# enricobottazzi/zk-fhe

Hardware: AMD Instinct MI355X
Metric: BFV proofs/sec (k=13) (higher is better)
Workload: dtype u32x8 (256-bit Montgomery integers over BN254 Fr/Fq)

## Files before the change

### zk-fhe_amd/csrc/msm.hip

```cpp
#include <cstdio>
#include <vector>
#include <cstring>

#include "ctx.hpp"
#include "fq29.hip.hpp"
#include "g1x29_wave.hip.hpp"

using namespace zk;

namespace {


__device__ __forceinline__ bool fr_gt_half(const Fr &s) {
  const u32 H[8] = {0xf8000000u, 0xa1f0fac9u, 0x3cdcb848u, 0x9419f424u, 0x40c0ac2eu, 0xdc2822dbu, 0x7098d014u, 0x18322739u};
#pragma unroll
  for (int i = 7; i >= 0; --i) {
    if (s.l[i] > H[i]) return true;
    if (s.l[i] < H[i]) return false;
  }
  return false;
}

struct Digits {
  int c, windows;
};

template <class F>
__device__ __forceinline__ void for_each_digit(const Fr &mont, int c, int windows, F f) {
  Fr s = fp_from_mont<FrP>(mont);
  bool neg = fr_gt_half(s);
  if (neg) s = fp_neg<FrP>(s);
  u32 carry = 0;
  const u32 mask = (1u << c) - 1, halfv = 1u << (c - 1);
  for (int w = 0; w < windows; ++w) {
    u32 v = (s.l[0] & mask) + carry;
#pragma unroll
    for (int i = 0; i < 7; ++i) s.l[i] = __builtin_amdgcn_alignbit(s.l[i + 1], s.l[i], (u32)c);
    s.l[7] >>= c;
    bool dneg = false;
    if (v > halfv) {
      v = (1u << c) - v;
      dneg = true;
      carry = 1;
    } else {
      carry = 0;
    }
    if (v) f(w, v, neg != dneg);
  }
}

constexpr size_t MSM_MAX_COLS = 4096;
constexpr unsigned SORT_CHUNK = 2048;
constexpr unsigned SORT_THREADS = 512;

__global__ void __launch_bounds__(SORT_THREADS) k_msm_hist(const Fr *__restrict__ scalars, size_t col_stride, size_t n, unsigned chunks_per_col, int c, int windows,
                                                          unsigned *__restrict__ hist , unsigned K1) {
  extern __shared__ unsigned lh[];
  const size_t col = blockIdx.x / chunks_per_col;
  const unsigned chunk = blockIdx.x % chunks_per_col;
  for (unsigned b = threadIdx.x; b < K1; b += SORT_THREADS) lh[b] = 0;
  __syncthreads();
  const size_t i0 = (size_t)chunk * SORT_CHUNK, i1 = min(n, i0 + SORT_CHUNK);
  for (size_t i = i0 + threadIdx.x; i < i1; i += SORT_THREADS)
    for_each_digit(scalars[col * col_stride + i], c, windows, [&](int, u32 b, bool) { atomicAdd(&lh[b], 1u); });
  __syncthreads();
  unsigned *h = hist + col * K1;
  for (unsigned b = threadIdx.x; b < K1; b += SORT_THREADS) {
    const unsigned v = lh[b];
    if (v) atomicAdd(&h[b], v);
  }
}

__global__ void __launch_bounds__(256) k_msm_scan(const unsigned *__restrict__ hist, unsigned *__restrict__ off,
                                                  unsigned *__restrict__ cursor, unsigned K1) {
  __shared__ unsigned part[256];
  const unsigned *h = hist + (size_t)blockIdx.x * K1;
  unsigned *o = off + (size_t)blockIdx.x * K1;
  unsigned *cu = cursor + (size_t)blockIdx.x * K1;
  const unsigned K = K1 - 1;
  const unsigned per = (K + 255) / 256;
  const unsigned lo = threadIdx.x * per, hi = min(lo + per, K);
  unsigned s = 0;
  for (unsigned b = lo; b < hi; ++b) s += h[b + 1];
  part[threadIdx.x] = s;
  __syncthreads();
  if (threadIdx.x == 0) {
    unsigned acc = 0;
    for (int i = 0; i < 256; ++i) {
      unsigned t = part[i];
      part[i] = acc;
      acc += t;
    }
  }
  __syncthreads();
  unsigned acc = part[threadIdx.x];
  for (unsigned b = lo; b < hi; ++b) {
    o[b] = acc;
    cu[b + 1] = acc;
    acc += h[b + 1];
  }
  if (hi == K) o[K] = acc;
}

__global__ void __launch_bounds__(SORT_THREADS) k_msm_scatter(const Fr *__restrict__ scalars, size_t col_stride, size_t n, unsigned chunks_per_col, int c, int windows,
                                                             unsigned *__restrict__ cursor, unsigned K1, unsigned *__restrict__ entries,
                                                             size_t col_entries) {
  extern __shared__ unsigned lh[];
  const size_t col = blockIdx.x / chunks_per_col;
  const unsigned chunk = blockIdx.x % chunks_per_col;
  for (unsigned b = threadIdx.x; b < K1; b += SORT_THREADS) lh[b] = 0;
  __syncthreads();
  const size_t i0 = (size_t)chunk * SORT_CHUNK, i1 = min(n, i0 + SORT_CHUNK);
  for (size_t i = i0 + threadIdx.x; i < i1; i += SORT_THREADS)
    for_each_digit(scalars[col * col_stride + i], c, windows, [&](int, u32 b, bool) { atomicAdd(&lh[b], 1u); });
  __syncthreads();
  unsigned *cu = cursor + col * K1;
  for (unsigned b = threadIdx.x; b < K1; b += SORT_THREADS) {
    const unsigned v = lh[b];
    lh[b] = v ? atomicAdd(&cu[b], v) : 0u;
  }
  __syncthreads();
  unsigned *e = entries + col * col_entries;
  for (size_t i = i0 + threadIdx.x; i < i1; i += SORT_THREADS)
    for_each_digit(scalars[col * col_stride + i], c, windows, [&](int w, u32 b, bool neg) {
      const unsigned pos = atomicAdd(&lh[b], 1u);
      e[pos] = ((unsigned)w * (unsigned)n + (unsigned)i) | (neg ? 0x80000000u : 0u);
    });
}

constexpr unsigned CH_SCALARS = 2048, CS_SCALARS = 512, CS_THREADS = 256, FINE_THREADS = 512, FINE_MAX = 256, FINE_COPIES = 8, FINE_CTRS = FINE_MAX * FINE_COPIES, FINE_TILE = 14336;
static_assert(FINE_CTRS == 4 * FINE_THREADS && FINE_TILE % (4 * FINE_THREADS) == 0, "k_msm_fine: four counters per thread, whole 16-byte loads per tile");
constexpr int FINE_BITS_MAX = 8;

__global__ void __launch_bounds__(CS_THREADS) k_msm_chist(const Fr *__restrict__ scalars, size_t col_stride, size_t n, unsigned chunks_per_col, int c, int windows,
                                                         int L, unsigned NB, unsigned *__restrict__ chist ) {
  extern __shared__ unsigned lh[];
  const size_t col = blockIdx.x / chunks_per_col;
  const unsigned chunk = blockIdx.x % chunks_per_col;
  for (unsigned b = threadIdx.x; b < NB; b += CS_THREADS) lh[b] = 0;
  __syncthreads();
  const size_t i0 = (size_t)chunk * CH_SCALARS, i1 = min(n, i0 + CH_SCALARS);
  for (size_t i = i0 + threadIdx.x; i < i1; i += CS_THREADS)
    for_each_digit(scalars[col * col_stride + i], c, windows, [&](int, u32 b, bool) { atomicAdd(&lh[(b - 1) >> L], 1u); });
  __syncthreads();
  for (unsigned g = threadIdx.x; g < NB; g += CS_THREADS) {
    const unsigned v = lh[g];
    if (v) atomicAdd(&chist[col * NB + g], v);
  }
}

__global__ void __launch_bounds__(64) k_msm_cscan(const unsigned *__restrict__ chist, unsigned NB, size_t n_cols, unsigned *__restrict__ coff ,
                                                  unsigned *__restrict__ ccursor ) {
  const size_t col = blockIdx.x * (size_t)blockDim.x + threadIdx.x;
  if (col >= n_cols) return;
  unsigned acc = 0;
  for (unsigned g = 0; g < NB; ++g) {
    coff[col * (NB + 1) + g] = acc;
    ccursor[col * NB + g] = acc;
    acc += chist[col * NB + g];
// ... 337 lines not shown
      const unsigned h = base + (lane >> 3), sub = lane & 7;
      size_t g = 0;
      unsigned nt = 0, pa = 0, pb = 0;
      Slices s = {0, 0, 0};
      if (h < cnt) {
        g = medium_list[h];
        const size_t col = g / K;
        const unsigned b = (unsigned)(g - col * K);
        const unsigned *o = off + col * (K + 1);
        s = slices_of(o[b + 1] - o[b], TASK_E);
        nt = s.nt;
        pa = bucket_posA[g];
        pb = bucket_posB[g];
      }
      G1X29 acc = G1X29::identity();
      for (unsigned j = sub; j < nt; j += 8) g1x29_add(acc, g1x29_load(partials[partial_pos(s, pa, pb, j)]));
      for (int m = 1; m < 8; m <<= 1) {
        const G1X29 other = g1x_shfl_xor(acc, m);
        g1x29_add(acc, other);
      }
      if (nt && sub == 0) buckets[g] = g1x29_store(acc);
    }
    return;
  }
  const unsigned first = large_blocks + medium_blocks, light_blocks = gridDim.x - first;
  const size_t total = (size_t)K * n_cols;
  for (size_t g = (blockIdx.x - first) * (size_t)blockDim.x + threadIdx.x; g < total; g += (size_t)light_blocks * blockDim.x) {
    const size_t col = g / K;
    const unsigned b = (unsigned)(g - col * K);
    const unsigned *o = off + col * (K + 1);
    const Slices s = slices_of(o[b + 1] - o[b], TASK_E);
    const unsigned nt = s.nt;
    if (nt > (unsigned)MERGE_LIGHT) continue;
    G1X first = G1X::identity();
    if (nt) {
      const unsigned pa = bucket_posA[g], pb = bucket_posB[g];
      first = partials[partial_pos(s, pa, pb, 0)];
      if (nt > 1) {
        G1X29 acc = g1x29_load(first);
        G1X nxt = partials[partial_pos(s, pa, pb, 1)];
        for (unsigned j = 1; j < nt; ++j) {
          const G1X cur = nxt;
          if (j + 1 < nt) nxt = partials[partial_pos(s, pa, pb, j + 1)];
          g1x29_add(acc, g1x29_load(cur));
        }
        first = g1x29_store(acc);
      }
    }
    buckets[g] = first;
  }
}

__device__ __forceinline__ G1X g1x_mul_pow2(G1X p, int k) {
  for (int i = 0; i < k; ++i) p = g1x_dbl(p);
  return p;
}
__device__ __forceinline__ G1X29 g1x29_mul_pow2(G1X29 p, int k) {
  for (int i = 0; i < k; ++i) p = g1x29_dbl(p);
  return p;
}

__global__ void __launch_bounds__(256) k_msm_marginals(const G1X *__restrict__ buckets, unsigned K, size_t n_cols, unsigned L ,
                                                       unsigned w0, unsigned w_cnt ,
                                                       G1X *__restrict__ marg ) {
  const unsigned A = K >> 6;
  const unsigned per_col = A + 64;
  const unsigned G = 64 / L;
  const size_t wave = (blockIdx.x * (size_t)blockDim.x + threadIdx.x) >> 6;
  const unsigned lane = threadIdx.x & 63, g = lane & (G - 1), sub = lane / G;
  const size_t o = wave * G + g;
  const bool live = o < n_cols * w_cnt;
  const size_t col = live ? o / w_cnt : 0;
  const unsigned w = w0 + (unsigned)(o - col * w_cnt);
  const G1X *B = buckets + col * K;
  size_t base, stride;
  unsigned cnt;
  if (w < A) {
    base = (size_t)w * 64 + sub;
    stride = L;
    cnt = 64 / L;
  } else {
    base = (size_t)sub * 64 + (w - A);
    stride = (size_t)L * 64;
    cnt = A > sub ? (A - sub + L - 1) / L : 0;
  }
  if (!live) cnt = 0;
  G1X29 v = G1X29::identity();
  for (unsigned i = 0; i < cnt; ++i) g1x29_add(v, g1x29_load(B[base + i * stride]));
  for (int m = (int)G; m < 64; m <<= 1) {
    const G1X29 other = g1x_shfl_xor(v, m);
    g1x29_add(v, other);
  }
  if (live && sub == 0) marg[col * per_col + w] = g1x29_store(v);
}

template <bool XYZZ>
__global__ void __launch_bounds__(576) k_msm_weighted(const G1X *__restrict__ marg, unsigned K, void *__restrict__ out) {
  __shared__ G1X sh[9];
  const unsigned A = K >> 6;
  const unsigned row_waves = (A + 63) / 64;
  const size_t col = blockIdx.x;
  const unsigned lane = threadIdx.x & 63, wv = threadIdx.x >> 6;
  const G1X *M = marg + col * (A + 64);
  const bool rows = wv < row_waves;
  const unsigned a = wv * 64 + lane;
  const G1X29 P = g1x29_load(rows ? (a < A ? M[a] : G1X::identity()) : M[A + lane]);
  const unsigned k = rows ? a : lane + 1;
  int nbits = 7;
  if (rows) {
    nbits = 0;
    while ((1u << nbits) < A) ++nbits;
  }
  G1X29 W = G1X29::identity();
  for (int bit = nbits - 1; bit >= 0; --bit) {
    W = g1x29_dbl(W);
    if ((k >> bit) & 1) g1x29_add(W, P);
  }
  if (rows) W = g1x29_mul_pow2(W, 6);
  for (int m = 1; m < 64; m <<= 1) {
    const G1X29 other = g1x_shfl_xor(W, m);
    g1x29_add(W, other);
  }
  if (lane == 0) sh[wv] = g1x29_store(W);
  __syncthreads();
  if (threadIdx.x == 0) {
    G1X29 t = g1x29_load(sh[0]);
    for (unsigned w = 1; w <= row_waves; ++w) g1x29_add(t, g1x29_load(sh[w]));
    if (XYZZ) ((G1X *)out)[col] = g1x29_to_std(t);
    else ((G1Affine *)out)[col] = g1x_to_affine(g1x29_to_std(t));
  }
}

template <bool XYZZ>
__global__ void __launch_bounds__(64) k_msm_small(const G1X *__restrict__ buckets, unsigned K, void *__restrict__ out) {
  const size_t col = blockIdx.x;
  const unsigned lane = threadIdx.x;
  const G1X29 P = g1x29_load(lane < K ? buckets[col * K + lane] : G1X::identity());
  const unsigned k = lane + 1;
  G1X29 W = G1X29::identity();
  for (int bit = 6; bit >= 0; --bit) {
    W = g1x29_dbl(W);
    if ((k >> bit) & 1) g1x29_add(W, P);
  }
  for (int m = 1; m < 64; m <<= 1) {
    const G1X29 other = g1x_shfl_xor(W, m);
    g1x29_add(W, other);
  }
  if (lane == 0) {
    if (XYZZ) ((G1X *)out)[col] = g1x29_to_std(W);
    else ((G1Affine *)out)[col] = g1x_to_affine(g1x29_to_std(W));
  }
}

struct BiasArg {
  u32 l[9];
};

__device__ __forceinline__ u32 bits_at(const u32 (&l)[9], int bit, int c) {
  const int limb = bit >> 5, sh = bit & 31;
  u32 lo = 0, hi = 0;
#pragma unroll
  for (int k = 0; k < 9; ++k) {
    if (k == limb) lo = l[k];
    if (k == limb + 1) hi = l[k];
  }
  return (u32)((((u64)hi << 32) | lo) >> sh) & ((1u << c) - 1);
}

__device__ __forceinline__ bool biased_scalar(const Fr &mont, const BiasArg &B, u32 (&out)[9], int &bits) {
  Fr s = fp_from_mont<FrP>(mont);
  const bool neg = fr_gt_half(s);
  if (neg) s = fp_neg<FrP>(s);
  bits = 0;
#pragma unroll
  for (int k = 0; k < 8; ++k)
    if (s.l[k]) bits = 32 * k + 32 - __clz(s.l[k]);
  u32 carry = 0;
#pragma unroll
  for (int k = 0; k < 8; ++k) {
    const u64 v = (u64)s.l[k] + B.l[k] + carry;
    out[k] = (u32)v;
    carry = (u32)(v >> 32);
  }
  out[8] = B.l[8] + carry;
  return neg;
}

__global__ void __launch_bounds__(64) k_basis_multiples(const G1Affine *__restrict__ bases, size_t n, int c, int W, G1Affine *__restrict__ T) {
  const size_t t = blockIdx.x * (size_t)blockDim.x + threadIdx.x;
  if (t >= n * (size_t)W) return;
  const size_t i = t / (size_t)W;
  const int w = (int)(t % (size_t)W);
  const size_t J = (size_t)1 << (c - 1);
  G1Affine *row = T + t * J;
  G1Affine b = bases[i];
  if (!b.is_identity() && w) b = g1x_to_affine(g1x_mul_pow2(g1x_from_affine(b), c * w));
  if (b.is_identity()) {
    for (size_t j = 0; j < J; ++j) row[j] = b;
    return;
  }
  row[0] = g1_affine_to_29(b);
  if (J == 1) return;
  G1X acc = g1x_from_affine_dbl(b);
  row[1] = g1_affine_to_29(g1x_to_affine(acc));
  for (size_t j = 2; j < J; ++j) {
    g1x_add_affine(acc, b, false);
    row[j] = g1_affine_to_29(g1x_to_affine(acc));
  }
}

template <bool TREE>
__global__ void __launch_bounds__(256, TREE ? 1 : 3) k_msm_table(const Fr *__restrict__ scalars, size_t col_stride, size_t n, const G1Affine *__restrict__ T, int c, int W, BiasArg B,
                                                   unsigned P, unsigned cpc , unsigned n_cols, unsigned max_part,
                                                   G1X *__restrict__ partials ,
                                                   unsigned *__restrict__ n_part ,
                                                   unsigned *__restrict__ col_next ,
                                                   unsigned *__restrict__ lists , unsigned long long *__restrict__ adds) {
  unsigned *__restrict__ lst = lists + (size_t)blockIdx.x * P * (unsigned)W;
  __shared__ G1X sh[TREE ? 128 : 1];
  __shared__ unsigned wave_cnt[4], item_sh;
  const unsigned lane = threadIdx.x & 63, wv = threadIdx.x >> 6;
  const int half = 1 << (c - 1);
  G1X29 acc = G1X29::identity();
  unsigned col = (unsigned)(((unsigned long long)blockIdx.x * n_cols) / gridDim.x), done = 0, total = 0;
  for (;;) {
    __syncthreads();
    if (threadIdx.x == 0) item_sh = atomicAdd(&col_next[col], 1u);
    __syncthreads();
    const unsigned chunk = item_sh;
    if (chunk >= cpc) {
      if (done) {
        if (TREE) acc = block_sum_256(acc, sh);
        __syncthreads();
        if (threadIdx.x == 0) item_sh = atomicAdd(&n_part[col], 1u);
        __syncthreads();
        const size_t slot = (size_t)col * max_part + item_sh;
        if (TREE) {
          if (threadIdx.x == 0) partials[slot] = g1x29_store(acc);
        } else {
          partials[slot * 256 + threadIdx.x] = g1x29_store(acc);
        }
        acc = G1X29::identity();
        done = 0;
      }
      __syncthreads();
      if (threadIdx.x == 0) item_sh = 0;
      __syncthreads();
      const unsigned MIN_JOIN = cpc < 4u ? cpc : 4u;
      unsigned best = 0;
      for (unsigned j = threadIdx.x; j < n_cols; j += 256) {
        const unsigned nx = __hip_atomic_load(&col_next[j], __ATOMIC_RELAXED, __HIP_MEMORY_SCOPE_AGENT);
        if (nx < cpc && (nx == 0 || cpc - nx >= MIN_JOIN)) {
          const unsigned h = ((j * 2654435761u) ^ (blockIdx.x * 40503u + 12345u) * 2246822519u) >> 13;
          best = max(best, (((h & 0x7ffffu) + 1u) << 12) | j);
        }
      }
      if (best) atomicMax(&item_sh, best);
      __syncthreads();
      const unsigned found = item_sh;
      if (!found) break;
      col = found & 4095u;
      continue;
    }
    ++done;
    {
      const size_t i = (size_t)chunk * P + threadIdx.x;
      const bool valid = threadIdx.x < P && i < n;
      u32 sb[9];
      bool neg = false;
      unsigned long long mask = 0;
      if (valid) {
        int bits;
        neg = biased_scalar(scalars[(size_t)col * col_stride + i], B, sb, bits);
        const int wtop = min(W, bits / c + 2);
        for (int w = 0; w < wtop; ++w)
          if ((int)bits_at(sb, w * c, c) != half) mask |= 1ull << w;
      }
      const unsigned mine = (unsigned)__popcll(mask);
      unsigned incl = mine;
#pragma unroll
      for (int d = 1; d < 64; d <<= 1) {
        const unsigned t = __shfl_up(incl, d);
        if ((int)lane >= d) incl += t;
      }
      if (lane == 63) wave_cnt[wv] = incl;
      __syncthreads();
      unsigned off = incl - mine;
      for (unsigned v = 0; v < wv; ++v) off += wave_cnt[v];
      const unsigned row0 = threadIdx.x * (unsigned)W;
      while (mask) {
        const int w = __builtin_ctzll(mask);
        mask &= mask - 1;
        const int d = (int)bits_at(sb, w * c, c) - half;
        lst[off++] = (((row0 + (unsigned)w) << (c - 1)) + (unsigned)(d < 0 ? -d : d) - 1u) | ((neg != (d < 0)) ? 0x80000000u : 0u);
      }
    }
    __syncthreads();
    const unsigned M = wave_cnt[0] + wave_cnt[1] + wave_cnt[2] + wave_cnt[3];
    total += M;
    const G1Affine *__restrict__ Tc = T + (((size_t)chunk * P * (size_t)W) << (c - 1));
    unsigned e = threadIdx.x, en = 0, en2 = 0;
    G1Affine p;
    if (e < M) {
      en = lst[e];
      p = Tc[en & 0x7fffffffu];
    }
    if (e + 256 < M) en2 = lst[e + 256];
    while (e < M) {
      const unsigned e2 = e + 256;
      unsigned en3 = 0;
      G1Affine p2;
      if (e2 < M) p2 = Tc[en2 & 0x7fffffffu];
      if (e2 + 256 < M) en3 = lst[e2 + 256];
      g1x29_add_affine(acc, g1a29_load(p), (en >> 31) != 0);
      e = e2;
      en = en2;
      en2 = en3;
      p = p2;
    }
  }
  if (adds && threadIdx.x == 0 && total) atomicAdd(adds, (unsigned long long)total);
}

template <bool XYZZ>
__global__ void __launch_bounds__(512) k_msm_table_fold(const G1X *__restrict__ partials, unsigned max_part, unsigned L, unsigned *__restrict__ n_part,
                                                        unsigned *__restrict__ col_next, void *__restrict__ out) {
  __shared__ G1X sh[256];
  const unsigned col = blockIdx.x, t = threadIdx.x & 255u, q = threadIdx.x >> 8;
  const unsigned np = n_part[col] * L;
  const G1X *mine = partials + (size_t)col * max_part * L;
  G1X29 f = G1X29::identity();
  {
    const unsigned first = L == 256 ? q * 256u + t : threadIdx.x, step = 512u;
    unsigned b = first;
    G1X cur;
    if (b < np) cur = mine[b];
    while (b < np) {
      const unsigned nb = b + step;
      G1X nxt;
      if (nb < np) nxt = mine[nb];
      g1x29_add(f, g1x29_load(cur));
      cur = nxt;
      b = nb;
    }
  }
  if (q == 1) sh[t] = g1x29_store(f);
  __syncthreads();
  if (q == 0) g1x29_add(f, g1x29_load(sh[t]));
  __syncthreads();
  if (q == 0 && t >= 128) sh[t - 128] = g1x29_store(f);
  __syncthreads();
  if (q == 0 && t < 128) g1x29_add(f, g1x29_load(sh[t]));
  __syncthreads();
  if (q == 0 && t >= 64 && t < 128) sh[t - 64] = g1x29_store(f);
  __syncthreads();
  if (threadIdx.x < 64) {
    g1x29_add(f, g1x29_load(sh[t]));
    for (int m = 1; m < 64; m <<= 1) {
      const G1X29 other = g1x_shfl_xor(f, m);
      g1x29_add(f, other);
    }
    if (threadIdx.x == 0) {
      if (XYZZ) ((G1X *)out)[col] = g1x29_to_std(f);
      else ((G1Affine *)out)[col] = g1x_to_affine(g1x29_to_std(f));
      n_part[col] = 0;
      col_next[col] = 0;
    }
  }
}

__global__ void __launch_bounds__(256) k_basis_table(const G1Affine *__restrict__ bases, size_t n, int c, int windows,
                                                     G1Affine *__restrict__ table) {
  const size_t i = blockIdx.x * (size_t)blockDim.x + threadIdx.x;
  if (i >= n) return;
  G1Affine p = bases[i];
  table[i] = g1_affine_to_29(p);
  G1X cur = g1x_from_affine(p);
  for (int w = 1; w < windows; ++w) {
    cur = g1x_mul_pow2(cur, c);
    G1Affine a = g1x_to_affine(cur);
    table[(size_t)w * n + i] = g1_affine_to_29(a);
    cur = g1x_from_affine(a);
  }
}

__global__ void __launch_bounds__(256) k_g1_add(const G1Affine *__restrict__ a, const G1Affine *__restrict__ b,
                                                G1Affine *__restrict__ out, size_t n) {
  const size_t i = blockIdx.x * (size_t)blockDim.x + threadIdx.x;
  if (i >= n) return;
  G1X acc = g1x_from_affine(a[i]);
  g1x_add_affine(acc, b[i], false);
  out[i] = g1x_to_affine(acc);
}

__global__ void __launch_bounds__(256) k_g1_mul(const G1Affine *__restrict__ p, const Fr *__restrict__ k,
                                                G1Affine *__restrict__ out, size_t n) {
  const size_t i = blockIdx.x * (size_t)blockDim.x + threadIdx.x;
  if (i >= n) return;
  const Fr s = fp_from_mont<FrP>(k[i]);
  const G1Affine base = p[i];
  G1X acc = G1X::identity();
  for (int bit = 255; bit >= 0; --bit) {
    acc = g1x_dbl(acc);
    if ((s.l[bit >> 5] >> (bit & 31)) & 1) g1x_add_affine(acc, base, false);
  }
  out[i] = g1x_to_affine(acc);
}

template <bool XYZZ>
__global__ void __launch_bounds__(64) k_msm_sparse(const zkfhe_sparse_term *__restrict__ terms, unsigned n_terms, const G1Affine *__restrict__ T, int c, int W,
                                                   BiasArg B, void *__restrict__ out) {
  const unsigned slot = blockIdx.x, lane = threadIdx.x;
  const int half = 1 << (c - 1);
  G1X29 acc = G1X29::identity();
  for (unsigned t = 0; t < n_terms; ++t) {
    if (terms[t].slot != slot) continue;
    Fr s;
#pragma unroll
    for (int i = 0; i < 4; ++i) {
      s.l[2 * i] = (u32)terms[t].scalar.l[i];
      s.l[2 * i + 1] = (u32)(terms[t].scalar.l[i] >> 32);
    }
    u32 sb[9];
    int bits;
    const bool neg = biased_scalar(s, B, sb, bits);
    const int d = (int)lane < W ? (int)bits_at(sb, (int)lane * c, c) - half : 0;
    if (d) {
      const G1Affine p = T[(((size_t)terms[t].row * W + lane) << (c - 1)) + (size_t)(d < 0 ? -d : d) - 1];
      g1x29_add_affine(acc, g1a29_load(p), neg != (d < 0));
    }
  }
  for (int m = 1; m < 64; m <<= 1) {
    const G1X29 other = g1x_shfl_xor(acc, m);
    g1x29_add(acc, other);
  }
  if (lane == 0) {
    if (XYZZ) ((G1X *)out)[slot] = g1x29_to_std(acc);
    else ((G1Affine *)out)[slot] = g1x_to_affine(g1x29_to_std(acc));
  }
}

int table_bits(size_t n, double budget_scale) {
  const char *e = getenv("ZKFHE_TABLE_BITS");
  const int forced = e ? atoi(e) : -1;
  const char *g = getenv("ZKFHE_TABLE_GB");
  double gb = g ? atof(g) : 48.0;
  if (!g) {
    size_t free_b = 0, total_b = 0;
    if (hipMemGetInfo(&free_b, &total_b) == hipSuccess && (double)free_b / 4.0 < gb * 1073741824.0) gb = (double)free_b / 4.0 / 1073741824.0;
  }
  const double budget = gb * 1073741824.0 * budget_scale;
  auto fits = [&](int c) {
    const double entries = (double)n * (double)((255 + c - 1) / c) * (double)(1u << (c - 1));
    return c >= 8 && c <= 15 && entries * sizeof(G1Affine) <= budget;
  };
  if (forced >= 0) return forced > 0 && fits(forced) ? forced : 0;
  for (int c = 15; c >= 8; --c)
    if (fits(c)) return c;
  return 0;
}

size_t table_reserve_bytes(size_t total_b) {
  if (const char *r = getenv("ZKFHE_TABLE_RESERVE_GB")) return (size_t)(atof(r) * 1073741824.0);
  const size_t eighth = total_b / 8, floor_b = (size_t)24 << 30;
  return eighth > floor_b ? eighth : floor_b;
}

BiasArg table_bias(int c, int W) {
  BiasArg B;
  memset(&B, 0, sizeof(B));
  for (int w = 0; w < W; ++w) {
    const int bit = c * w + c - 1;
    B.l[bit >> 5] |= 1u << (bit & 31);
  }
  return B;
}

int msm_table(zkfhe_ctx *ctx, const zkfhe_basis *basis, const Fr *scalars, size_t col_stride, size_t n_cols, void *out, bool xyzz) {
  const size_t n = basis->n;
  const int c = basis->mc, W = basis->mw;
  const size_t words = 2 * MSM_MAX_COLS + 4;
  if (!ctx->tickets) {
    ZK_HIP(ctx, hipMalloc((void **)&ctx->tickets, words * sizeof(unsigned)));
    ZK_HIP(ctx, zk_memset_async(ctx, ctx->tickets, 0, words * sizeof(unsigned), ctx->stream));
  }
  unsigned *n_part = ctx->tickets, *col_next = ctx->tickets + MSM_MAX_COLS;
  unsigned long long *adds = (unsigned long long *)(ctx->tickets + 2 * MSM_MAX_COLS);
  const size_t grid_max = (size_t)ctx->num_cu * 3;
  size_t P = 256;
  while (P > 128 && n_cols * ((n + P - 1) / P) < grid_max) P >>= 1;
  const size_t cpc = (n + P - 1) / P, n_items = n_cols * cpc;
  const size_t grid = n_items < grid_max ? n_items : grid_max;
  const size_t max_part = cpc < grid ? cpc : grid;
  const bool tree = n_cols <= 16;
  const unsigned L = tree ? 1 : 256;
  void *p0, *p1;
  int rc = zk_scratch(ctx, 0, n_cols * max_part * L * sizeof(G1X), &p0);
  if (rc) return rc;
  rc = zk_scratch(ctx, 1, grid * P * (size_t)W * 4, &p1);
  if (rc) return rc;
  const bool big = n_cols * n > ((size_t)1 << 16);
  const int slot = big ? 0 : 2;
  if (ctx->prof_on) ZK_HIP(ctx, zk_memset_async(ctx, adds, 0, 8, ctx->stream));
  zk_prof_begin(ctx);
  if (tree)
    k_msm_table<true><<<(unsigned)grid, 256, 0, ctx->stream>>>(scalars, col_stride, n, basis->mult, c, W, table_bias(c, W), (unsigned)P, (unsigned)cpc, (unsigned)n_cols,
                                                             (unsigned)max_part, (G1X *)p0, n_part, col_next, (unsigned *)p1, ctx->prof_on ? adds : nullptr);
  else
    k_msm_table<false><<<(unsigned)grid, 256, 0, ctx->stream>>>(scalars, col_stride, n, basis->mult, c, W, table_bias(c, W), (unsigned)P, (unsigned)cpc, (unsigned)n_cols,
                                                              (unsigned)max_part, (G1X *)p0, n_part, col_next, (unsigned *)p1, ctx->prof_on ? adds : nullptr);
  ZK_LAUNCH_CHECK(ctx);
  zk_prof_end(ctx, slot, 96.0 * (double)n * (double)n_cols);
  {
    static const bool dbg = getenv("ZKFHE_DEBUG_NPART") != nullptr;
    if (dbg) {
      std::vector<unsigned> np(n_cols);
      ZK_HIP(ctx, hipMemcpy(np.data(), n_part, n_cols * sizeof(unsigned), hipMemcpyDeviceToHost));
      unsigned long long sum = 0;
      unsigned mx = 0;
      for (unsigned v : np) {
        sum += v;
        mx = v > mx ? v : mx;
      }
      fprintf(stderr, "[msm_table] cols %zu  chunks/col %zu  grid %zu  visits/col avg %.1f max %u\n", n_cols, cpc, grid, (double)sum / n_cols, mx);
    }
  }
  if (xyzz) k_msm_table_fold<true><<<(unsigned)n_cols, 512, 0, ctx->stream>>>((const G1X *)p0, (unsigned)max_part, L, n_part, col_next, out);
  else k_msm_table_fold<false><<<(unsigned)n_cols, 512, 0, ctx->stream>>>((const G1X *)p0, (unsigned)max_part, L, n_part, col_next, out);
  ZK_LAUNCH_CHECK(ctx);
  if (ctx->prof_on) {
    unsigned long long h = 0;
    ZK_HIP(ctx, hipMemcpy(&h, adds, 8, hipMemcpyDeviceToHost));
    ctx->prof_ops[slot] += (double)h;
  }
  return ZKFHE_OK;
}

static unsigned two_level_min_k() {
  const char *e = getenv("ZKFHE_SORT");
  return e && e[0] == '2' ? 2048u : 16384u;
}

int default_window_bits(size_t n) {
  if (n <= 64) return 5;
  if (n <= 1024) return 8;
  if (n <= 4096) return 11;
  if (n <= 16384) return 13;
  if (n <= 131072) return 14;
  return 16;
}

}

extern "C" {

int zkfhe_basis_create(zkfhe_ctx *ctx, const zkfhe_g1_affine *bases_host, size_t n, int window_bits, zkfhe_basis **out) {
  return zk_basis_create_scaled(ctx, bases_host, n, window_bits, 1.0, out);
}

}

int zk_basis_create_scaled(zkfhe_ctx *ctx, const zkfhe_g1_affine *bases_host, size_t n, int window_bits, double table_budget_scale, zkfhe_basis **out) {
  ZK_ENTER(ctx);
  ZK_ARG(ctx, out != nullptr && bases_host != nullptr && n > 0);
  ZK_ARG(ctx, window_bits == 0 || (window_bits >= 2 && window_bits <= 16));
  const int c = window_bits ? window_bits : default_window_bits(n);
  const int windows = (254 + c - 1) / c;
  ZK_ARG(ctx, (size_t)windows * n < ((size_t)1 << 31));
  zkfhe_basis *b = new zkfhe_basis();
  b->n = n;
  b->c = c;
  b->windows = windows;
  hipError_t e = hipMalloc((void **)&b->table, (size_t)windows * n * sizeof(G1Affine));
  if (e != hipSuccess) {
    delete b;
    return zk_fail(ctx, e == hipErrorOutOfMemory ? ZKFHE_ENOMEM : ZKFHE_EHIP, "hipMalloc(basis table)", e, __FILE__, __LINE__);
  }
  void *tmp;
  int rc = zk_scratch(ctx, 0, n * sizeof(G1Affine), &tmp);
  if (rc) return rc;
  ZK_HIP(ctx, zk_memcpy_async(ctx, tmp, bases_host, n * sizeof(G1Affine), hipMemcpyHostToDevice, ctx->stream));
  k_basis_table<<<zk_blocks(n, 256), 256, 0, ctx->stream>>>((const G1Affine *)tmp, n, c, windows, b->table);
  ZK_LAUNCH_CHECK(ctx);
  int mc = window_bits == 0 && n >= 256 ? table_bits(n, table_budget_scale) : 0;
  const int mc_budget = mc;
  bool narrowed = false;
  for (; mc >= 8; --mc) {
    const int mw = (255 + mc - 1) / mc;
    const size_t bytes = (n * (size_t)mw << (mc - 1)) * sizeof(G1Affine);
    size_t free_b = 0, total_b = 0;
    if (hipMemGetInfo(&free_b, &total_b) != hipSuccess || free_b < bytes + table_reserve_bytes(total_b)) {
      narrowed = true;
      continue;
    }
    e = hipMalloc((void **)&b->mult, bytes);
    if (e != hipSuccess) {
      (void)hipGetLastError();
      b->mult = nullptr;
      narrowed = true;
      continue;
    }
    b->mc = mc;
    b->mw = mw;
    b->mult_bytes = bytes;
    k_basis_multiples<<<zk_blocks(n * (size_t)mw, 64), 64, 0, ctx->stream>>>((const G1Affine *)tmp, n, mc, mw, b->mult);
    ZK_LAUNCH_CHECK(ctx);
    break;
  }
  ZK_HIP(ctx, hipStreamSynchronize(ctx->stream));
  b->narrowed = narrowed && b->mc < mc_budget;
  if (getenv("ZKFHE_VERBOSE"))
    fprintf(stderr, "[zkfhe] basis n = %zu: digit-multiple table %d bits, %.1f GB resident%s\n", n, b->mc, (double)b->mult_bytes / 1073741824.0,
            b->narrowed ? " (narrower than the budget allows: the device did not have the room)" : (b->mc ? "" : " (none: bucket pipeline)"));
  *out = b;
  return ZKFHE_OK;
}

extern "C" {

int zkfhe_basis_destroy(zkfhe_ctx *ctx, zkfhe_basis *basis) {
  ZK_ENTER(ctx);
  if (!basis) return ZKFHE_OK;
  ZK_HIP(ctx, hipStreamSynchronize(ctx->stream));
  hipFree(basis->table);
  if (basis->mult) hipFree(basis->mult);
  delete basis;
  return ZKFHE_OK;
}

size_t zkfhe_basis_len(const zkfhe_basis *basis) { return basis ? basis->n : 0; }

int zkfhe_msm_batch(zkfhe_ctx *ctx, const zkfhe_basis *basis, const zkfhe_fr *scalars_dev, size_t n_cols, zkfhe_g1_affine *out_dev) {
  return zk_msm_batch_strided(ctx, basis, scalars_dev, basis ? basis->n : 0, n_cols, out_dev);
}

int zkfhe_msm_batch_xyzz(zkfhe_ctx *ctx, const zkfhe_basis *basis, const zkfhe_fr *scalars_dev, size_t n_cols, zkfhe_g1_xyzz *out_dev) {
  return zk_msm_batch_strided_form(ctx, basis, scalars_dev, basis ? basis->n : 0, n_cols, out_dev, true);
}

}

int zk_msm_batch_strided(zkfhe_ctx *ctx, const zkfhe_basis *basis, const zkfhe_fr *scalars_dev, size_t col_stride, size_t n_cols, zkfhe_g1_affine *out_dev) {
  return zk_msm_batch_strided_form(ctx, basis, scalars_dev, col_stride, n_cols, out_dev, false);
}

int zk_msm_batch_strided_form(zkfhe_ctx *ctx, const zkfhe_basis *basis, const zkfhe_fr *scalars_dev, size_t col_stride, size_t n_cols, void *out_dev, bool xyzz) {
  ZK_ENTER(ctx);
  ZK_ARG(ctx, basis != nullptr);
  if (!n_cols) return ZKFHE_OK;
  ZK_ARG(ctx, scalars_dev != nullptr && out_dev != nullptr && col_stride >= basis->n);
  const size_t n = basis->n;
  ZK_ARG(ctx, n_cols <= MSM_MAX_COLS);
  static const char *wide_env = getenv("ZKFHE_TABLE_WIDE");
  const bool wide = wide_env ? wide_env[0] == '1' : basis->mw <= basis->windows + 2;
  if (basis->mult && (wide || n_cols <= 8))
    return msm_table(ctx, basis, (const Fr *)scalars_dev, col_stride, n_cols, out_dev, xyzz);
  const int c = basis->c, W = basis->windows;
  const unsigned K = 1u << (c - 1), K1 = K + 1;
  const size_t col_entries = n * (size_t)W;
  const unsigned TASK_E = task_len(col_entries, K);
  const size_t max_tasks = (n_cols * col_entries) / TASK_E + (size_t)K * n_cols;
  const size_t heavy_cap = (n_cols * col_entries) / ((size_t)TASK_E * MERGE_LIGHT) + 1;
  const size_t words = 3 * n_cols * K1 + 2 * (size_t)K * n_cols + 2 * n_cols * TASK_BINS + 16 + 2 * heavy_cap + 2 * max_tasks;
  void *p1, *p2, *p0;
  int rc = zk_scratch(ctx, 1, words * sizeof(unsigned), &p1);
  if (rc) return rc;
  rc = zk_scratch(ctx, 2, n_cols * col_entries * sizeof(unsigned) + 64, &p2);
  if (rc) return rc;
  int idx_bits = 1;
  while (((size_t)1 << idx_bits) < col_entries) ++idx_bits;
  int L = 31 - idx_bits;
  if (L > FINE_BITS_MAX) L = FINE_BITS_MAX;
  const char *sort_env = getenv("ZKFHE_SORT");
  if (sort_env && sort_env[0] == '2' && sort_env[1] == ':' && atoi(sort_env + 2) >= 6 && atoi(sort_env + 2) < L) L = atoi(sort_env + 2);
  const bool two_level = K >= two_level_min_k() && L >= 6 && !(sort_env && sort_env[0] == '1');
  const unsigned NB = two_level ? K >> L : 0;
  size_t s0 = (n_cols * (size_t)K + max_tasks) * sizeof(G1X);
  const size_t stage_stride = (col_entries + 3) & ~(size_t)3;
// ... 183 lines not shown
```

Baseline: 268.9.

## Specialize MSM table digit extraction on window width and use 29-bit Montgomery reduction

```diff
diff --git a/zk-fhe_amd/csrc/msm.hip b/zk-fhe_amd/csrc/msm.hip
--- a/zk-fhe_amd/csrc/msm.hip
+++ b/zk-fhe_amd/csrc/msm.hip
@@ -5,6 +5,7 @@
 #include "ctx.hpp"
 #include "fq29.hip.hpp"
 #include "g1x29_wave.hip.hpp"
+#include "msm_digits.hip.hpp"
 
 using namespace zk;
 
@@ -648,39 +649,6 @@
   }
 }
 
-struct BiasArg {
-  u32 l[9];
-};
-
-__device__ __forceinline__ u32 bits_at(const u32 (&l)[9], int bit, int c) {
-  const int limb = bit >> 5, sh = bit & 31;
-  u32 lo = 0, hi = 0;
-#pragma unroll
-  for (int k = 0; k < 9; ++k) {
-    if (k == limb) lo = l[k];
-    if (k == limb + 1) hi = l[k];
-  }
-  return (u32)((((u64)hi << 32) | lo) >> sh) & ((1u << c) - 1);
-}
-
-__device__ __forceinline__ bool biased_scalar(const Fr &mont, const BiasArg &B, u32 (&out)[9], int &bits) {
-  Fr s = fp_from_mont<FrP>(mont);
-  const bool neg = fr_gt_half(s);
-  if (neg) s = fp_neg<FrP>(s);
-  bits = 0;
-#pragma unroll
-  for (int k = 0; k < 8; ++k)
-    if (s.l[k]) bits = 32 * k + 32 - __clz(s.l[k]);
-  u32 carry = 0;
-#pragma unroll
-  for (int k = 0; k < 8; ++k) {
-    const u64 v = (u64)s.l[k] + B.l[k] + carry;
-    out[k] = (u32)v;
-    carry = (u32)(v >> 32);
-  }
-  out[8] = B.l[8] + carry;
-  return neg;
-}
 
 __global__ void __launch_bounds__(64) k_basis_multiples(const G1Affine *__restrict__ bases, size_t n, int c, int W, G1Affine *__restrict__ T) {
   const size_t t = blockIdx.x * (size_t)blockDim.x + threadIdx.x;
@@ -705,18 +673,14 @@
   }
 }
 
-template <bool TREE>
-__global__ void __launch_bounds__(256, TREE ? 1 : 3) k_msm_table(const Fr *__restrict__ scalars, size_t col_stride, size_t n, const G1Affine *__restrict__ T, int c, int W, BiasArg B,
-                                                   unsigned P, unsigned cpc , unsigned n_cols, unsigned max_part,
-                                                   G1X *__restrict__ partials ,
-                                                   unsigned *__restrict__ n_part ,
-                                                   unsigned *__restrict__ col_next ,
-                                                   unsigned *__restrict__ lists , unsigned long long *__restrict__ adds) {
+template <bool TREE, int C>
+__device__ __forceinline__ void msm_table_body(const Fr *__restrict__ scalars, size_t col_stride, size_t n, const G1Affine *__restrict__ T, int c_arg, int W, const BiasArg &B,
+                                               unsigned P, unsigned cpc, unsigned n_cols, unsigned max_part, G1X *__restrict__ partials, unsigned *__restrict__ n_part,
+                                               unsigned *__restrict__ col_next, unsigned *__restrict__ lists, unsigned long long *__restrict__ adds, G1X *sh,
+                                               unsigned (&wave_cnt)[4], unsigned &item_sh) {
   unsigned *__restrict__ lst = lists + (size_t)blockIdx.x * P * (unsigned)W;
-  __shared__ G1X sh[TREE ? 128 : 1];
-  __shared__ unsigned wave_cnt[4], item_sh;
   const unsigned lane = threadIdx.x & 63, wv = threadIdx.x >> 6;
-  const int half = 1 << (c - 1);
+  const int c = C ? C : c_arg;
   G1X29 acc = G1X29::identity();
   unsigned col = (unsigned)(((unsigned long long)blockIdx.x * n_cols) / gridDim.x), done = 0, total = 0;
   for (;;) {
@@ -762,17 +726,8 @@
     {
       const size_t i = (size_t)chunk * P + threadIdx.x;
       const bool valid = threadIdx.x < P && i < n;
-      u32 sb[9];
-      bool neg = false;
-      unsigned long long mask = 0;
-      if (valid) {
-        int bits;
-        neg = biased_scalar(scalars[(size_t)col * col_stride + i], B, sb, bits);
-        const int wtop = min(W, bits / c + 2);
-        for (int w = 0; w < wtop; ++w)
-          if ((int)bits_at(sb, w * c, c) != half) mask |= 1ull << w;
-      }
-      const unsigned mine = (unsigned)__popcll(mask);
+      MsmDigits<C> D;
+      const unsigned mine = msm_digits<C>(valid, scalars + ((size_t)col * col_stride + i), B, c, W, D);
       unsigned incl = mine;
 #pragma unroll
       for (int d = 1; d < 64; d <<= 1) {
@@ -783,17 +738,14 @@
       __syncthreads();
       unsigned off = incl - mine;
       for (unsigned v = 0; v < wv; ++v) off += wave_cnt[v];
-      const unsigned row0 = threadIdx.x * (unsigned)W;
-      while (mask) {
-        const int w = __builtin_ctzll(mask);
-        mask &= mask - 1;
-        const int d = (int)bits_at(sb, w * c, c) - half;
-        lst[off++] = (((row0 + (unsigned)w) << (c - 1)) + (unsigned)(d < 0 ? -d : d) - 1u) | ((neg != (d < 0)) ? 0x80000000u : 0u);
-      }
+      unsigned row0 = threadIdx.x * (unsigned)W;
+      asm volatile("" : "+v"(row0));
+      msm_emit<C>(D, c, row0, [&](u32 entry) { lst[off++] = entry; });
     }
     __syncthreads();
     const unsigned M = wave_cnt[0] + wave_cnt[1] + wave_cnt[2] + wave_cnt[3];
     total += M;
+    if (adds && threadIdx.x == 0 && M) atomicAdd(adds + 1, (unsigned long long)((M + 255u) & ~255u));
     const G1Affine *__restrict__ Tc = T + (((size_t)chunk * P * (size_t)W) << (c - 1));
     unsigned e = threadIdx.x, en = 0, en2 = 0;
     G1Affine p;
@@ -816,6 +768,20 @@
     }
   }
   if (adds && threadIdx.x == 0 && total) atomicAdd(adds, (unsigned long long)total);
+}
+
+template <bool TREE>
+__global__ void __launch_bounds__(256, TREE ? 1 : 3) k_msm_table(const Fr *__restrict__ scalars, size_t col_stride, size_t n, const G1Affine *__restrict__ T, int c, int W, BiasArg B,
+                                                   unsigned P, unsigned cpc , unsigned n_cols, unsigned max_part,
+                                                   G1X *__restrict__ partials ,
+                                                   unsigned *__restrict__ n_part ,
+                                                   unsigned *__restrict__ col_next ,
+                                                   unsigned *__restrict__ lists , unsigned long long *__restrict__ adds ) {
+  __shared__ G1X sh[TREE ? 128 : 1];
+  __shared__ unsigned wave_cnt[4], item_sh;
+  if (c == 15) msm_table_body<TREE, 15>(scalars, col_stride, n, T, c, W, B, P, cpc, n_cols, max_part, partials, n_part, col_next, lists, adds, sh, wave_cnt, item_sh);
+  else if (c == 13) msm_table_body<TREE, 13>(scalars, col_stride, n, T, c, W, B, P, cpc, n_cols, max_part, partials, n_part, col_next, lists, adds, sh, wave_cnt, item_sh);
+  else msm_table_body<TREE, 0>(scalars, col_stride, n, T, c, W, B, P, cpc, n_cols, max_part, partials, n_part, col_next, lists, adds, sh, wave_cnt, item_sh);
 }
 
 template <bool XYZZ>
@@ -997,29 +963,32 @@
   if (rc) return rc;
   const bool big = n_cols * n > ((size_t)1 << 16);
   const int slot = big ? 0 : 2;
-  if (ctx->prof_on) ZK_HIP(ctx, zk_memset_async(ctx, adds, 0, 8, ctx->stream));
+  static const bool dbg = getenv("ZKFHE_DEBUG_NPART") != nullptr;
+  const bool count = ctx->prof_on || dbg;
+  if (count) ZK_HIP(ctx, zk_memset_async(ctx, adds, 0, 16, ctx->stream));
   zk_prof_begin(ctx);
   if (tree)
     k_msm_table<true><<<(unsigned)grid, 256, 0, ctx->stream>>>(scalars, col_stride, n, basis->mult, c, W, table_bias(c, W), (unsigned)P, (unsigned)cpc, (unsigned)n_cols,
-                                                             (unsigned)max_part, (G1X *)p0, n_part, col_next, (unsigned *)p1, ctx->prof_on ? adds : nullptr);
+                                                             (unsigned)max_part, (G1X *)p0, n_part, col_next, (unsigned *)p1, count ? adds : nullptr);
   else
     k_msm_table<false><<<(unsigned)grid, 256, 0, ctx->stream>>>(scalars, col_stride, n, basis->mult, c, W, table_bias(c, W), (unsigned)P, (unsigned)cpc, (unsigned)n_cols,
-                                                              (unsigned)max_part, (G1X *)p0, n_part, col_next, (unsigned *)p1, ctx->prof_on ? adds : nullptr);
+                                                              (unsigned)max_part, (G1X *)p0, n_part, col_next, (unsigned *)p1, count ? adds : nullptr);
   ZK_LAUNCH_CHECK(ctx);
   zk_prof_end(ctx, slot, 96.0 * (double)n * (double)n_cols);
-  {
-    static const bool dbg = getenv("ZKFHE_DEBUG_NPART") != nullptr;
-    if (dbg) {
-      std::vector<unsigned> np(n_cols);
-      ZK_HIP(ctx, hipMemcpy(np.data(), n_part, n_cols * sizeof(unsigned), hipMemcpyDeviceToHost));
-      unsigned long long sum = 0;
-      unsigned mx = 0;
-      for (unsigned v : np) {
-        sum += v;
-        mx = v > mx ? v : mx;
-      }
-      fprintf(stderr, "[msm_table] cols %zu  chunks/col %zu  grid %zu  visits/col avg %.1f max %u\n", n_cols, cpc, grid, (double)sum / n_cols, mx);
-    }
+  if (dbg) {
+    std::vector<unsigned> np(n_cols);
+    unsigned long long h[2] = {0, 0};
+    ZK_HIP(ctx, hipStreamSynchronize(ctx->stream));
+    ZK_HIP(ctx, hipMemcpy(np.data(), n_part, n_cols * sizeof(unsigned), hipMemcpyDeviceToHost));
+    ZK_HIP(ctx, hipMemcpy(h, adds, 16, hipMemcpyDeviceToHost));
+    unsigned long long sum = 0;
+    unsigned mx = 0;
+    for (unsigned v : np) {
+      sum += v;
+      mx = v > mx ? v : mx;
+    }
+    fprintf(stderr, "[msm_table] cols %zu  chunks/col %zu  grid %zu  visits/col avg %.1f max %u  entries %llu  issued lane-additions %llu (%.3f per entry)\n", n_cols, cpc,
+            grid, (double)sum / n_cols, mx, h[0], h[1], h[0] ? (double)h[1] / (double)h[0] : 0.0);
   }
   if (xyzz) k_msm_table_fold<true><<<(unsigned)n_cols, 512, 0, ctx->stream>>>((const G1X *)p0, (unsigned)max_part, L, n_part, col_next, out);
   else k_msm_table_fold<false><<<(unsigned)n_cols, 512, 0, ctx->stream>>>((const G1X *)p0, (unsigned)max_part, L, n_part, col_next, out);
diff --git a/zk-fhe_amd/csrc/msm_digits.hip.hpp b/zk-fhe_amd/csrc/msm_digits.hip.hpp
--- /dev/null
+++ b/zk-fhe_amd/csrc/msm_digits.hip.hpp
@@ -0,0 +1,158 @@
+#pragma once
+#include "fr29.hip.hpp"
+
+namespace zk {
+
+struct BiasArg {
+  u32 l[9];
+};
+
+ZK_HD u32 bits_at(const u32 (&l)[9], int bit, int c) {
+  const int limb = bit >> 5, sh = bit & 31;
+  u32 lo = 0, hi = 0;
+#pragma unroll
+  for (int k = 0; k < 9; ++k) {
+    if (k == limb) lo = l[k];
+    if (k == limb + 1) hi = l[k];
+  }
+  return (u32)((((u64)hi << 32) | lo) >> sh) & ((1u << c) - 1);
+}
+
+ZK_HD Fr msm_from_mont(const Fr &w) {
+  constexpr u32 P[9] = ZK_R29_P;
+  u32 t[9], m[9];
+  t[0] = (w.l[0] << 5) & q29::MASK;
+#pragma unroll
+  for (int i = 1; i < 9; ++i) {
+    const int bit = 29 * i - 5, k = bit >> 5, sh = bit & 31;
+    u32 v = w.l[k] >> sh;
+    if (sh > 3 && k + 1 < 8) v |= w.l[k + 1] << (32 - sh);
+    t[i] = v & q29::MASK;
+  }
+  F29 r;
+  u64 acc = 0;
+#pragma unroll
+  for (int k = 0; k < 17; ++k) {
+    if (k < 9) acc += t[k];
+#pragma unroll
+    for (int j = (k < 9 ? 0 : k - 8); j <= (k < 9 ? k - 1 : 8); ++j) acc += (u64)m[j] * P[k - j];
+    if (k < 9) {
+      m[k] = ((u32)acc * r29::INV) & q29::MASK;
+      acc += (u64)m[k] * P[0];
+    } else {
+      r.l[k - 9] = (u32)acc & q29::MASK;
+    }
+    acc >>= 29;
+  }
+  r.l[8] = (u32)acc;
+  return fr29_pack(r);
+}
+
+ZK_HD bool biased_scalar(const Fr &mont, const BiasArg &B, u32 (&out)[9], int &bits) {
+  Fr s = msm_from_mont(mont);
+  const u32 H[8] = {0xf8000000u, 0xa1f0fac9u, 0x3cdcb848u, 0x9419f424u, 0x40c0ac2eu, 0xdc2822dbu, 0x7098d014u, 0x18322739u};
+  u32 bh = 0, bn = 0, n[8];
+#pragma unroll
+  for (int k = 0; k < 8; ++k) {
+    (void)zk_subc(H[k], s.l[k], bh, &bh);
+    n[k] = zk_subc(FrP::MOD[k], s.l[k], bn, &bn);
+  }
+  const bool neg = bh != 0;
+#pragma unroll
+  for (int k = 0; k < 8; ++k) s.l[k] = neg ? n[k] : s.l[k];
+  bits = 0;
+#pragma unroll
+  for (int k = 0; k < 8; ++k)
+    if (s.l[k]) bits = 32 * k + 32 - __builtin_clz(s.l[k]);
+  u32 carry = 0;
+#pragma unroll
+  for (int k = 0; k < 8; ++k) {
+    const u64 v = (u64)s.l[k] + B.l[k] + carry;
+    out[k] = (u32)v;
+    carry = (u32)(v >> 32);
+  }
+  out[8] = B.l[8] + carry;
+  return neg;
+}
+
+ZK_HD bool msm_any_lane(bool p) {
+#if defined(__HIP_DEVICE_COMPILE__)
+  return __builtin_amdgcn_ballot_w64(p) != 0;
+#else
+  return p;
+#endif
+}
+
+template <int C>
+struct MsmDigits {
+  static constexpr int MAXW = C ? (255 + C - 1) / C : 32;
+  u32 sb[9];
+  int wtop;
+  bool neg;
+};
+
+template <int C, class F>
+ZK_HD void msm_for_each_window(const MsmDigits<C> &D, int c_arg, F f) {
+  const int c = C ? C : c_arg;
+  const u32 cmask = (1u << c) - 1;
+  const int half = 1 << (c - 1);
+  if constexpr (C != 0) {
+#pragma unroll
+    for (int w = 0; w < MsmDigits<C>::MAXW; ++w) {
+      const bool in = w < D.wtop;
+      if (!msm_any_lane(in)) break;
+      const int bit = C * w, k = bit >> 5, s = bit & 31;
+      u32 v = D.sb[k] >> s;
+      if (s + C > 32) v |= D.sb[k + 1] << (32 - s);
+      f(w, in ? (int)(v & cmask) - half : 0);
+    }
+  } else {
+    u32 sh[9];
+#pragma unroll
+    for (int k = 0; k < 9; ++k) sh[k] = D.sb[k];
+#pragma unroll
+    for (int w = 0; w < MsmDigits<C>::MAXW; ++w) {
+      const bool in = w < D.wtop;
+      if (!msm_any_lane(in)) break;
+      const u32 v = sh[0] & cmask;
+#pragma unroll
+      for (int k = 0; k < 8; ++k) sh[k] = (sh[k] >> c) | (sh[k + 1] << (32 - c));
+      sh[8] >>= c;
+      f(w, in ? (int)v - half : 0);
+    }
+  }
+}
+
+template <int C>
+ZK_HD unsigned msm_digits(bool have, const Fr *scalar, const BiasArg &B, int c_arg, int W, MsmDigits<C> &D) {
+  const int c = C ? C : c_arg;
+#pragma unroll
+  for (int k = 0; k < 9; ++k) D.sb[k] = 0;
+  D.wtop = 0;
+  D.neg = false;
+  if (have) {
+    const Fr mont = *scalar;
+    u32 any = 0;
+#pragma unroll
+    for (int k = 0; k < 8; ++k) any |= mont.l[k];
+    if (any) {
+      int bits;
+      D.neg = biased_scalar(mont, B, D.sb, bits);
+      const int wt = bits / c + 2;
+      D.wtop = wt < W ? wt : W;
+    }
+  }
+  unsigned count = 0;
+  msm_for_each_window<C>(D, c, [&](int, int d) { count += d != 0; });
+  return count;
+}
+
+template <int C, class F>
+ZK_HD void msm_emit(const MsmDigits<C> &D, int c_arg, unsigned row0, F f) {
+  const int c = C ? C : c_arg;
+  msm_for_each_window<C>(D, c, [&](int w, int d) {
+    if (d) f((((row0 + (unsigned)w) << (c - 1)) + (unsigned)(d < 0 ? -d : d) - 1u) | ((D.neg != (d < 0)) ? 0x80000000u : 0u));
+  });
+}
+
+}
```

After: 266.4. About the same (-0.9%).
